# Deci-AI/super-gradients

Measured on NVIDIA H100. Metric: images/sec YOLO-NAS-S 640 bf16 train, higher is better.
Workload: dtype bf16

## Files before the change

super_gradients_b200/csrc/conv_sm100.cu:

```cuda
#include <cuda.h>

#include <cstdio>
#include <cstdlib>
#include <cstring>

#include "common.cuh"
#include "conv_sm100.h"
#include "sm100_host.h"
#include "sm100_ptx.cuh"

namespace sm100 {

constexpr int BLOCK_M = 128;
constexpr int NUM_THREADS = 384;
constexpr int CONSUMER_THREADS = 256;
constexpr int MAX_STAGES = 8;

struct Params {
  int M;
  int N;
  int C;
  int KC;
  int n_tiles;
  int stages;
  int P, Q;
  int stride, pad;
  int b_cols_per_tap;
  int ntaps;
  signed char tap_dh[9], tap_dw[9], tap_b[9];
  int out_mode, o_mul, oh_add, ow_add, outH, outW;
  int halo_tw, halo_thw;
  long long y_pitch;
  int y_off;
  bf16* y;
  const float* scale;
  const float* shift;
  const bf16* residual;
  double* stats;
  int stats_repl;
  int act;
// ... 206 lines not shown
        wgmma_commit();
        if (prev >= 0) {
          wgmma_wait<1>();
          __syncwarp();
          if (lane == 0) mbar_arrive(empty_bar(prev));
        }
        prev = stg;
        if (++stg == p.stages) {
          stg = 0;
          par ^= 1;
        }
      }
      wgmma_wait<0>();
      fence_regs(acc);
      __syncwarp();
      if (lane == 0 && prev >= 0) mbar_arrive(empty_bar(prev));

      const long long m_lo = (long long)mt * BLOCK_M + wg * 64 + wq * 16 + (lane >> 2);
      long long orow[2];
      bool row_ok[2];
#pragma unroll
      for (int h = 0; h < 2; ++h) {
        const long long m = m_lo + 8 * h;
        row_ok[h] = m < p.M;
        orow[h] = out_row(p, row_ok[h] ? m : 0);
      }
      tile_epilogue<BN>(p, acc, orow, row_ok, nt, wg, wq, lane, s_part, s_stats);
    }
  }
  __syncthreads();
  flush_stats(p, s_stats);
}

constexpr int HALO_W = 10, HALO_H = 10, HALO_TILE = 8;
constexpr uint32_t HALO_CG_BYTES = 1664;
constexpr uint32_t HALO_CTRL_BYTES = CTRL_BAR_BYTES + 16;
constexpr int HALO_MAX_STAGES = 6;

template <int BN, bool SKIP>
__global__ void __launch_bounds__(NUM_THREADS, BN <= 48 ? 2 : 1)
conv3x3_halo_kernel(const __grid_constant__ CUtensorMap map_a, const __grid_constant__ CUtensorMap map_b, const Params p) {
  extern __shared__ __align__(1024) unsigned char smem_raw[];
  const uint32_t smem_base = (smem_u32(smem_raw) + 1023u) & ~1023u;
  const int ksteps = p.C / 16;
  constexpr uint32_t b_box = BN * 32;
  const uint32_t b_bytes = 9u * ksteps * b_box;
  const uint32_t a_stage = ((uint32_t)(p.C / 8) * HALO_CG_BYTES + 1023u) & ~1023u;
  const uint32_t sb = smem_base, sa0 = smem_base + ((b_bytes + 1023u) & ~1023u);
  const uint32_t ctrl = sa0 + p.stages * a_stage;
  auto full_bar = [&](int s) { return ctrl + 8u * s; };
  auto empty_bar = [&](int s) { return ctrl + 8u * (MAX_STAGES + s); };
  const uint32_t b_bar = ctrl + CTRL_BAR_BYTES;
  float* s_part = reinterpret_cast<float*>(smem_raw + (ctrl + HALO_CTRL_BYTES - smem_u32(smem_raw)));
  float* s_stats = s_part + 8 * 2 * BN;

  const int warp = threadIdx.x >> 5, lane = threadIdx.x & 31;
  const int m_tiles = p.M;
  const int nt = blockIdx.x % p.n_tiles;
  const int mt_step = gridDim.x / p.n_tiles;
  const int mt0 = blockIdx.x / p.n_tiles;
  const int off = SKIP ? off_centre_steps<BN>(p, nt, ksteps, 16) : ksteps;

  if (threadIdx.x == 0) {
    for (int s = 0; s < p.stages; ++s) {
      mbar_init(full_bar(s), 1);
      mbar_init(empty_bar(s), 4);
    }
    mbar_init(b_bar, 1);
    asm volatile("fence.mbarrier_init.release.cluster;" ::: "memory");
    asm volatile("fence.proxy.async.shared::cta;" ::: "memory");
  }
  if (p.stats)
    for (int i = threadIdx.x; i < 4 * p.N; i += NUM_THREADS) s_stats[i] = 0.f;
  __syncthreads();

  if (warp == 0) {
    if (elect_one()) {
      mbar_expect_tx(b_bar, (uint32_t)(8 * off + ksteps) * b_box);
      for (int bt = 0; bt < 9; ++bt)
        for (int ks = 0; ks < (bt == CENTRE_TAP ? ksteps : off); ++ks)
          tma_load_2d(sb + (uint32_t)(bt * ksteps + ks) * b_box, &map_b, b_bar, bt * p.b_cols_per_tap + 16 * ks, nt * BN);
      const uint32_t a_tx = (uint32_t)(p.C / 8) * (HALO_H * HALO_W * 16);
      int stg = 0;
      uint32_t par = 1;
      for (int mt = mt0; mt < m_tiles; mt += mt_step) {
        const int n_img = mt / p.halo_thw;
        const int rem = mt - n_img * p.halo_thw;
        const int th = rem / p.halo_tw, tw = rem - th * p.halo_tw;
        mbar_wait(empty_bar(stg), par);
        const uint32_t sa = sa0 + stg * a_stage;
        mbar_expect_tx(full_bar(stg), a_tx);
        for (int cg = 0; cg < p.C / 8; ++cg)
          tma_load_tiled_4d(sa + (uint32_t)cg * HALO_CG_BYTES, &map_a, full_bar(stg), 8 * cg, tw * HALO_TILE - 1, th * HALO_TILE - 1,
                            n_img);
        if (++stg == p.stages) {
          stg = 0;
          par ^= 1;
        }
      }
    }
  } else if (warp >= 4) {
    const int wg = (warp >> 2) - 1;
    const int wq = warp & 3;
    float acc[BN / 2];
    mbar_wait(b_bar, 0);
    for (int j = wg, mt = mt0 + wg * mt_step; mt < m_tiles; j += 2, mt += 2 * mt_step) {
      const int stg = j % p.stages;
      mbar_wait(full_bar(stg), (uint32_t)(j / p.stages) & 1u);
      const uint32_t sa = sa0 + stg * a_stage;
      wgmma_fence();
      int t = off > 0 ? 0 : CENTRE_TAP;
      uint32_t sa_t = sa + (uint32_t)((t / 3) * HALO_W + t % 3) * 16u, sb_t = sb + (uint32_t)(p.tap_b[t] * ksteps) * b_box;
      for (int k = 0, ks = 0, nk = 8 * off + ksteps; k < nk; ++k) {
        const uint64_t da = smem_desc_noswizzle(sa_t + (uint32_t)(2 * ks) * HALO_CG_BYTES, HALO_CG_BYTES, HALO_W * 16);
        const uint64_t db = smem_desc(sb_t + (uint32_t)ks * b_box, 32, 16u, 256u);
        mma_kk<BN>(acc, da, db, k != 0);
        if (++ks == (t == CENTRE_TAP ? ksteps : off) && ++t < 9) {
          ks = 0;
          sa_t = sa + (uint32_t)((t / 3) * HALO_W + t % 3) * 16u;
          sb_t = sb + (uint32_t)(p.tap_b[t] * ksteps) * b_box;
        }
      }
      wgmma_commit();
      wgmma_wait<0>();
      fence_regs(acc);
      __syncwarp();
      if (lane == 0) mbar_arrive(empty_bar(stg));

      const int n_img = mt / p.halo_thw;
      const int rem = mt - n_img * p.halo_thw;
      const int th = rem / p.halo_tw, tw = rem - th * p.halo_tw;
      const int ow = tw * HALO_TILE + (lane >> 2);
      long long orow[2];
      bool row_ok[2];
#pragma unroll
      for (int h = 0; h < 2; ++h) {
        const int oh = th * HALO_TILE + 2 * wq + h;
        row_ok[h] = oh < p.P && ow < p.Q;
        orow[h] = row_ok[h] ? ((long long)n_img * p.P + oh) * p.Q + ow : 0;
      }
      tile_epilogue<BN, 4>(p, acc, orow, row_ok, nt, wg, wq, lane, s_part + wg * 4 * 2 * BN, s_stats + wg * 2 * p.N);
    }
  }
  __syncthreads();
  if (p.stats) {
    for (int i = threadIdx.x; i < 2 * p.N; i += NUM_THREADS) s_stats[i] += s_stats[2 * p.N + i];
    __syncthreads();
  }
  flush_stats(p, s_stats);
}

struct WParams {
// ... 103 lines not shown
        wgmma_commit();
        if (prev >= 0) {
          wgmma_wait<1>();
          __syncwarp();
          if (lane == 0) mbar_arrive(empty_bar(prev));
        }
        prev = stg;
        if ((stg += it_step) >= p.stages) {
          stg -= p.stages;
          par ^= 1;
        }
      }
      if (prev < 0) return;
      wgmma_wait<0>();
      fence_regs(acc);
      const int row_len = p.R * p.S * p.cpad;
#pragma unroll
      for (int h = 0; h < 2; ++h) {
        const int ko = row0 + (shared_rows ? 0 : wg * 64) + wq * 16 + (lane >> 2) + 8 * h;
        if (ko < p.K) {
          float* drow = p.dw + (long long)ko * row_len + tap * p.cpad + ctile * NB + 2 * (lane & 3);
#pragma unroll
          for (int j = 0; j < NB / 8; ++j)
            asm volatile("red.global.add.v2.f32 [%0], {%1, %2};" ::"l"(drow + 8 * j), "f"(acc[4 * j + 2 * h]), "f"(acc[4 * j + 2 * h + 1])
                         : "memory");
        }
      }
    }
  }
}

constexpr uint32_t WH_A_BYTES = WPIX * 128;

__host__ __device__ constexpr uint32_t wgrad_halo_stage_bytes(int nb) {
  return (WH_A_BYTES + (uint32_t)(nb / 8) * HALO_CG_BYTES + 1023u) & ~1023u;
}

template <int NB, int NT>
__device__ __forceinline__ void wgrad_halo_consume(const WParams& p, uint32_t ring, uint32_t bars, int t0, int t1, int tap0, int rb,
                                                   int ctile) {
  constexpr uint32_t stage_bytes = wgrad_halo_stage_bytes(NB);
  const int wq = (threadIdx.x >> 5) & 3, lane = threadIdx.x & 31;
  auto full_bar = [&](int s) { return bars + 8u * s; };
  auto empty_bar = [&](int s) { return bars + 8u * (MAX_STAGES + s); };
  float acc[NT > 0 ? NT : 1][NB / 2];
  int stg = 0, prev = 0;
  uint32_t par = 0;
  for (int mt = t0; mt < t1; ++mt) {
    mbar_wait(full_bar(stg), par);
    if constexpr (NT > 0) {
      const uint32_t sa = ring + stg * stage_bytes, sx = sa + WH_A_BYTES;
      wgmma_fence();
#pragma unroll
      for (int t = 0; t < NT; ++t) {
        const int tap = tap0 + t;
        const uint32_t sx_t = sx + (uint32_t)((tap / 3) * HALO_W + tap % 3) * 16u;
#pragma unroll
        for (int j = 0; j < WPIX / 16; ++j) {
          const uint64_t da = smem_desc(sa + (uint32_t)j * 16u * 128u, 128, WPIX * 128, 8 * 128);
          const uint64_t db = smem_desc_noswizzle(sx_t + (uint32_t)j * 2u * HALO_W * 16u, HALO_W * 16, HALO_CG_BYTES);
          mma_mn<NB>(acc[t], da, db, (mt != t0 || j != 0) ? 1u : 0u);
        }
      }
      wgmma_commit();
      wgmma_wait<1>();
    }
    __syncwarp();
    if (lane == 0 && mt != t0) mbar_arrive(empty_bar(prev));
    prev = stg;
    if (++stg == p.stages) {
      stg = 0;
      par ^= 1;
    }
  }
  if constexpr (NT > 0) {
    wgmma_wait<0>();
#pragma unroll
    for (int t = 0; t < NT; ++t) fence_regs(acc[t]);
  }
  __syncwarp();
  if (lane == 0) mbar_arrive(empty_bar(prev));
  if constexpr (NT > 0) {
    const int row_len = 9 * p.cpad;
#pragma unroll
    for (int h = 0; h < 2; ++h) {
      const int ko = 64 * rb + wq * 16 + (lane >> 2) + 8 * h;
      if (ko < p.K) {
        float* drow = p.dw + (long long)ko * row_len + tap0 * p.cpad + ctile * NB + 2 * (lane & 3);
#pragma unroll
        for (int t = 0; t < NT; ++t)
#pragma unroll
          for (int j = 0; j < NB / 8; ++j)
            asm volatile("red.global.add.v2.f32 [%0], {%1, %2};" ::"l"(drow + t * p.cpad + 8 * j), "f"(acc[t][4 * j + 2 * h]),
                         "f"(acc[t][4 * j + 2 * h + 1])
                         : "memory");
      }
    }
  }
}

template <int NB>
__global__ void __launch_bounds__(NUM_THREADS, 1)
wgrad3x3_halo_kernel(const __grid_constant__ CUtensorMap map_dy, const __grid_constant__ CUtensorMap map_x, const WParams p) {
  extern __shared__ __align__(1024) unsigned char smem_raw[];
  const uint32_t smem_base = (smem_u32(smem_raw) + 1023u) & ~1023u;
  constexpr uint32_t a_bytes = WH_A_BYTES, stage_bytes = wgrad_halo_stage_bytes(NB);
  const uint32_t ctrl = smem_base + p.stages * stage_bytes;
  auto full_bar = [&](int s) { return ctrl + 8u * s; };
  auto empty_bar = [&](int s) { return ctrl + 8u * (MAX_STAGES + s); };

  const int warp = threadIdx.x >> 5;
  const int items = p.rb_all * p.n_ctiles;
  const int split = blockIdx.x / items, item = blockIdx.x - split * items;
  const int ctile = item / p.rb_all, rb = item - ctile * p.rb_all;
  const bool all_taps = rb < p.rb_off;
  const int t0 = split * p.tiles_per_cta, t1 = min(t0 + p.tiles_per_cta, p.tiles);

  if (threadIdx.x == 0) {
    for (int s = 0; s < p.stages; ++s) {
      mbar_init(full_bar(s), 1);
      mbar_init(empty_bar(s), 8);
    }
    asm volatile("fence.mbarrier_init.release.cluster;" ::: "memory");
    asm volatile("fence.proxy.async.shared::cta;" ::: "memory");
  }
  __syncthreads();

  if (warp == 0) {
    if (elect_one()) {
      const uint32_t tx = a_bytes + (NB / 8) * (HALO_H * HALO_W * 16);
      int stg = 0;
      uint32_t par = 1;
      for (int mt = t0; mt < t1; ++mt) {
        const int n_img = mt / p.halo_thw;
        const int rem = mt - n_img * p.halo_thw;
        const int th = rem / p.halo_tw, tw = rem - th * p.halo_tw;
        mbar_wait(empty_bar(stg), par);
        const uint32_t sa = smem_base + stg * stage_bytes;
        mbar_expect_tx(full_bar(stg), tx);
        tma_load_tiled_4d(sa, &map_dy, full_bar(stg), 64 * rb, tw * HALO_TILE, th * HALO_TILE, n_img);
        for (int cg = 0; cg < NB / 8; ++cg)
          tma_load_tiled_4d(sa + a_bytes + (uint32_t)cg * HALO_CG_BYTES, &map_x, full_bar(stg), ctile * NB + 8 * cg,
                            tw * HALO_TILE - 1, th * HALO_TILE - 1, n_img);
        if (++stg == p.stages) {
          stg = 0;
          par ^= 1;
        }
      }
    }
  } else if (warp >= 4) {
    const int wg = (warp >> 2) - 1;
    const uint32_t ring = smem_base, bars = ctrl;
    if (!all_taps && wg == 0)
      wgrad_halo_consume<NB, 1>(p, ring, bars, t0, t1, CENTRE_TAP, rb, ctile);
    else if (!all_taps)
      wgrad_halo_consume<NB, 0>(p, ring, bars, t0, t1, 0, rb, ctile);
    else if (wg == 0)
      wgrad_halo_consume<NB, 5>(p, ring, bars, t0, t1, 0, rb, ctile);
    else
      wgrad_halo_consume<NB, 4>(p, ring, bars, t0, t1, 5, rb, ctile);
  }
}

typedef CUresult (*EncodeTiledFn)(CUtensorMap*, CUtensorMapDataType, cuuint32_t, void*, const cuuint64_t*, const cuuint64_t*,
                                  const cuuint32_t*, const cuuint32_t*, CUtensorMapInterleave, CUtensorMapSwizzle,
                                  CUtensorMapL2promotion, CUtensorMapFloatOOBfill);
typedef CUresult (*EncodeIm2colFn)(CUtensorMap*, CUtensorMapDataType, cuuint32_t, void*, const cuuint64_t*, const cuuint64_t*,
                                   const int*, const int*, cuuint32_t, cuuint32_t, const cuuint32_t*, CUtensorMapInterleave,
                                   CUtensorMapSwizzle, CUtensorMapL2promotion, CUtensorMapFloatOOBfill);
EncodeTiledFn g_tiled = nullptr;
EncodeIm2colFn g_im2col = nullptr;
int g_num_sms = 0;
long long g_launches = 0;
long long g_halo_launches = 0;
long long g_wgrad_halo_launches = 0;
bool g_force_im2col = false;
bool g_wgrad_force_im2col = false;
long long launch_count() { return g_launches; }
long long halo_launch_count() { return g_halo_launches; }
long long wgrad_halo_launch_count() { return g_wgrad_halo_launches; }
void force_im2col(bool on) { g_force_im2col = on; }
void wgrad_force_im2col(bool on) { g_wgrad_force_im2col = on; }

int init_driver() {
  if (g_tiled && g_im2col) return SGB_OK;
  cudaDriverEntryPointQueryResult qres;
  void* fn = nullptr;
  if (cudaGetDriverEntryPoint("cuTensorMapEncodeTiled", &fn, cudaEnableDefault, &qres) != cudaSuccess || !fn) {
    sgb_set_error("cuTensorMapEncodeTiled entry point not found");
    return SGB_E_CUDA;
  }
  g_tiled = (EncodeTiledFn)fn;
  fn = nullptr;
  if (cudaGetDriverEntryPoint("cuTensorMapEncodeIm2col", &fn, cudaEnableDefault, &qres) != cudaSuccess || !fn) {
    sgb_set_error("cuTensorMapEncodeIm2col entry point not found");
    return SGB_E_CUDA;
  }
  g_im2col = (EncodeIm2colFn)fn;
  int dev = 0;
  cudaGetDevice(&dev);
  cudaDeviceGetAttribute(&g_num_sms, cudaDevAttrMultiProcessorCount, dev);
  return SGB_OK;
}

int encode_tiled(CUtensorMap* map, const void* ptr, int rank, const cuuint64_t* dims, const cuuint64_t* byte_strides,
                 const cuuint32_t* box, CUtensorMapSwizzle swizzle, const char* what) {
  const cuuint32_t elem_strides[5] = {1, 1, 1, 1, 1};
  const CUresult r = g_tiled(map, CU_TENSOR_MAP_DATA_TYPE_BFLOAT16, (cuuint32_t)rank, const_cast<void*>(ptr), dims, byte_strides, box,
                             elem_strides, CU_TENSOR_MAP_INTERLEAVE_NONE, swizzle, CU_TENSOR_MAP_L2_PROMOTION_L2_128B,
                             CU_TENSOR_MAP_FLOAT_OOB_FILL_NONE);
  if (r == CUDA_SUCCESS) return SGB_OK;
  char shape[256] = "";
  for (int i = 0, n = 0; i < rank && n < (int)sizeof(shape); ++i)
    n += snprintf(shape + n, sizeof(shape) - n, "%s%llu (box %u, stride %llu)", i ? ", " : "", (unsigned long long)dims[i],
                  (unsigned)box[i], i ? (unsigned long long)byte_strides[i - 1] : 2ull);
  sgb_set_error("cuTensorMapEncodeTiled(%s) failed with %d: dims %s", what, (int)r, shape);
  return SGB_E_CUDA;
}

namespace {

CUtensorMapSwizzle swizzle_for(int kc) {
  return kc == 64 ? CU_TENSOR_MAP_SWIZZLE_128B : (kc == 32 ? CU_TENSOR_MAP_SWIZZLE_64B : CU_TENSOR_MAP_SWIZZLE_32B);
}

int encode_im2col(CUtensorMap* map, const void* ptr, int N, int H, int W, int C, int pitch, int stride, const int (&lower)[2],
                  const int (&upper)[2], int channels, int pixels, const char* what) {
  const cuuint64_t dims[4] = {(cuuint64_t)C, (cuuint64_t)W, (cuuint64_t)H, (cuuint64_t)N};
  const cuuint64_t strides[3] = {(cuuint64_t)pitch * 2, (cuuint64_t)W * pitch * 2, (cuuint64_t)H * W * pitch * 2};
  const cuuint32_t estr[4] = {1, (cuuint32_t)stride, (cuuint32_t)stride, 1};
  const CUresult r = g_im2col(map, CU_TENSOR_MAP_DATA_TYPE_BFLOAT16, 4, const_cast<void*>(ptr), dims, strides, lower, upper,
                              (cuuint32_t)channels, (cuuint32_t)pixels, estr, CU_TENSOR_MAP_INTERLEAVE_NONE, swizzle_for(channels),
                              CU_TENSOR_MAP_L2_PROMOTION_L2_128B, CU_TENSOR_MAP_FLOAT_OOB_FILL_NONE);
  if (r == CUDA_SUCCESS) return SGB_OK;
  sgb_set_error("cuTensorMapEncodeIm2col(%s) failed with %d (C=%d W=%d H=%d N=%d pitch=%d lower=%d,%d upper=%d,%d stride=%d box=%d)", what,
                (int)r, C, W, H, N, pitch, lower[0], lower[1], upper[0], upper[1], stride, channels);
  return SGB_E_CUDA;
}

int encode_halo_map(CUtensorMap* map, const void* x, int N, int H, int W, int C, int pitch) {
  const cuuint64_t dims[4] = {(cuuint64_t)C, (cuuint64_t)W, (cuuint64_t)H, (cuuint64_t)N};
  const cuuint64_t strides[3] = {(cuuint64_t)pitch * 2, (cuuint64_t)W * pitch * 2, (cuuint64_t)H * W * pitch * 2};
  const cuuint32_t box[4] = {8, HALO_W, HALO_H, 1};
  return encode_tiled(map, x, 4, dims, strides, box, CU_TENSOR_MAP_SWIZZLE_NONE, "halo");
}

struct Problem {
  const void* a;
  int N, H, W, C, a_pitch;
  const void* b;
  int b_rows, b_cols, b_cols_per_tap;
  int R, S, stride, pad, P, Q, flip;
  int ntaps;
  int tap_dh[9], tap_dw[9], tap_b[9];
  int out_mode, o_mul, oh_add, ow_add, outH, outW;
  void* y;
  int y_pitch, y_off;
  const float* scale;
  const float* shift;
  const void* residual;
  double* stats;
  int stats_repl, act;
  int centre_from;
};

bool supported(const Problem& q) {
  if (q.C % 16 != 0 || q.b_rows % 8 != 0) return false;
  if (!((q.R == 1 && q.S == 1) || (q.R == 3 && q.S == 3))) return false;
  if (q.stride != 1 && q.stride != 2) return false;
  if (q.a_pitch % 8 != 0 || q.y_pitch % 8 != 0 || q.y_off % 8 != 0) return false;
  if (((uintptr_t)q.a & 15) || ((uintptr_t)q.b & 15) || ((uintptr_t)q.y & 15)) return false;
  if ((long long)q.N * q.P * q.Q >= (1ll << 31)) return false;
  if (q.b_rows > 4096) return false;
  return true;
}

template <class Fn>
struct Variant {
  int bn;
  Fn fn;
  int regs = 0;
  bool ready = false;
};
typedef void (*ConvFn)(const CUtensorMap, const CUtensorMap, const Params);
typedef void (*WgradFn)(const CUtensorMap, const CUtensorMap, const WParams);
template <bool SKIP>
Variant<ConvFn> g_conv[6] = {{16, conv_wgmma_kernel<16, SKIP>}, {32, conv_wgmma_kernel<32, SKIP>},
                             {48, conv_wgmma_kernel<48, SKIP>}, {64, conv_wgmma_kernel<64, SKIP>},
                             {96, conv_wgmma_kernel<96, SKIP>}, {128, conv_wgmma_kernel<128, SKIP>}};
template <bool SKIP>
Variant<ConvFn> g_halo[6] = {{16, conv3x3_halo_kernel<16, SKIP>}, {32, conv3x3_halo_kernel<32, SKIP>},
                             {48, conv3x3_halo_kernel<48, SKIP>}, {64, conv3x3_halo_kernel<64, SKIP>},
                             {96, conv3x3_halo_kernel<96, SKIP>}, {128, conv3x3_halo_kernel<128, SKIP>}};
Variant<WgradFn> g_wgrad[6] = {{16, wgrad_wgmma_kernel<16>}, {32, wgrad_wgmma_kernel<32>}, {48, wgrad_wgmma_kernel<48>},
                               {64, wgrad_wgmma_kernel<64>}, {96, wgrad_wgmma_kernel<96>}, {128, wgrad_wgmma_kernel<128>}};
Variant<WgradFn> g_wgrad_halo[3] = {{16, wgrad3x3_halo_kernel<16>}, {32, wgrad3x3_halo_kernel<32>}, {48, wgrad3x3_halo_kernel<48>}};

template <class Fn, int N>
int prepare(Variant<Fn> (&table)[N], int bn, const char* what, Variant<Fn>*& var) {
  for (auto& v : table)
    if (v.bn == bn) var = &v;
  if (var->ready) return SGB_OK;
  if (int rc = sgb_cuda_check(cudaFuncSetAttribute(var->fn, cudaFuncAttributeMaxDynamicSharedMemorySize, 227 * 1024), what)) return rc;
  cudaFuncAttributes fa{};
  if (int rc = sgb_cuda_check(cudaFuncGetAttributes(&fa, var->fn), what)) return rc;
  var->regs = fa.numRegs;
  var->ready = true;
  return SGB_OK;
}

int max_ctas_per_sm(int regs) {
  const int ctas = 65536 / (((regs + 7) / 8) * 8 * NUM_THREADS);
  return ctas > 2 ? 2 : (ctas < 1 ? 1 : ctas);
}

int pick_bn(int n) {
  for (int bn : {16, 32, 48, 64, 96, 128})
    if (n <= bn) return bn;
  int best = 128, best_waste = (n + 127) / 128 * 128 - n;
  for (int bn : {96, 64}) {
    const int waste = (n + bn - 1) / bn * bn - n;
    if (waste < best_waste) { best_waste = waste; best = bn; }
  }
  return best;
}

size_t halo_smem(int C, int bn, int n, bool stats, int stages) {
  const size_t b_bytes = ((size_t)9 * C * bn * 2 + 1023) & ~(size_t)1023;
  const size_t a_stage = ((size_t)(C / 8) * HALO_CG_BYTES + 1023) & ~(size_t)1023;
  return 1024 + b_bytes + (size_t)stages * a_stage + HALO_CTRL_BYTES + (stats ? (size_t)(8 * 2 * bn + 4 * n) * 4 : 0);
}

bool halo_tiles_fit(int P, int Q) {
  const long long covered = (long long)((P + 7) / 8) * 8 * ((Q + 7) / 8) * 8;
  return 20ll * P * Q >= 17 * covered;
}

int halo_bn(const Problem& q) {
  if (q.R != 3 || q.S != 3 || q.stride != 1 || q.pad != 1 || q.ntaps > 0 || q.out_mode != 0) return 0;
  if (q.P != q.H || q.Q != q.W) return 0;
  if (!halo_tiles_fit(q.P, q.Q)) return 0;
  const int n = q.b_rows, full = pick_bn(n);
  auto waste = [&](int bn) { return (n + bn - 1) / bn * bn - n; };
  for (int bn : {full, 96, 64})
    if (bn <= full && (bn == full || (q.C <= 96 && bn >= 64 && waste(bn) <= waste(full))) &&
        halo_smem(q.C, bn, n, q.stats != nullptr, 2) <= 227 * 1024)
      return bn;
  return 0;
}

int launch_halo(const Problem& q, const Params& p0, int bn, cudaStream_t st) {
  Params p = p0;
  p.n_tiles = (p.N + bn - 1) / bn;
  p.halo_tw = (q.Q + HALO_TILE - 1) / HALO_TILE;
  p.halo_thw = p.halo_tw * ((q.P + HALO_TILE - 1) / HALO_TILE);
  p.M = q.N * p.halo_thw;
  p.centre_n = 0;
  Variant<ConvFn>* var = nullptr;
  if (int rc = prepare(p.centre_c > 0 ? g_halo<true> : g_halo<false>, bn, "conv3x3_halo_kernel", var)) return rc;
  int ctas_per_sm = max_ctas_per_sm(var->regs);
  int stages = 0;
  for (;; --ctas_per_sm) {
    const size_t budget = (ctas_per_sm == 1 ? 227u : 227u / ctas_per_sm - 1u) * 1024u;
    for (stages = HALO_MAX_STAGES; stages >= 2 && halo_smem(q.C, bn, p.N, p.stats != nullptr, stages) > budget; --stages) {
    }
    if (stages >= 2 || ctas_per_sm == 1) break;
  }
  if (stages < 2) { sgb_set_error("conv3x3_halo: tile does not fit shared memory"); return SGB_E_UNSUPPORTED; }
  p.stages = stages;
  const size_t smem = halo_smem(q.C, bn, p.N, p.stats != nullptr, stages);

  alignas(64) CUtensorMap map_a, map_b;
  if (int rc = encode_halo_map(&map_a, q.a, q.N, q.H, q.W, q.C, q.a_pitch)) return rc;
  const cuuint64_t b_dims[2] = {(cuuint64_t)q.b_cols, (cuuint64_t)q.b_rows}, b_strides[1] = {(cuuint64_t)q.b_cols * 2};
  const cuuint32_t b_box[2] = {16, (cuuint32_t)bn};
  if (int rc = encode_tiled(&map_b, q.b, 2, b_dims, b_strides, b_box, CU_TENSOR_MAP_SWIZZLE_32B, "halo B")) return rc;
  int per_nt = g_num_sms * ctas_per_sm / p.n_tiles;
  if (per_nt > p.M) per_nt = p.M;
  if (per_nt < 1) per_nt = 1;
  var->fn<<<per_nt * p.n_tiles, NUM_THREADS, smem, st>>>(map_a, map_b, p);
  ++g_launches;
  ++g_halo_launches;
  return sgb_cuda_check(cudaGetLastError(), "conv3x3_halo_kernel");
}

int launch(const Problem& q, cudaStream_t st) {
  if (int rc = init_driver()) return rc;
  Params p{};
  p.M = q.N * q.P * q.Q;
  p.N = q.b_rows;
  p.C = q.C;
  p.KC = q.C % 64 == 0 ? 64 : (q.C % 32 == 0 ? 32 : 16);
  if (p.KC < 64 && q.C > 32) p.KC = 64;
  const int bn = pick_bn(p.N);
  p.n_tiles = (p.N + bn - 1) / bn;
  p.P = q.P; p.Q = q.Q; p.stride = q.stride; p.pad = q.pad;
  if (q.ntaps > 0) {
    p.ntaps = q.ntaps;
    for (int t = 0; t < q.ntaps; ++t) { p.tap_dh[t] = (signed char)q.tap_dh[t]; p.tap_dw[t] = (signed char)q.tap_dw[t]; p.tap_b[t] = (signed char)q.tap_b[t]; }
  } else {
    p.ntaps = q.R * q.S;
    for (int t = 0; t < p.ntaps; ++t) {
      p.tap_dh[t] = (signed char)(t / q.S);
      p.tap_dw[t] = (signed char)(t % q.S);
      p.tap_b[t] = (signed char)(q.flip ? (p.ntaps - 1 - t) : t);
    }
  }
  if (p.ntaps > 9) return SGB_E_UNSUPPORTED;
  p.out_mode = q.out_mode; p.o_mul = q.o_mul; p.oh_add = q.oh_add; p.ow_add = q.ow_add; p.outH = q.outH; p.outW = q.outW;
  p.b_cols_per_tap = q.b_cols_per_tap;
  p.y = (bf16*)q.y; p.y_pitch = q.y_pitch; p.y_off = q.y_off;
  p.scale = q.scale; p.shift = q.shift; p.residual = (const bf16*)q.residual;
  p.stats = q.stats; p.stats_repl = q.stats_repl > 0 ? q.stats_repl : 1; p.act = q.act;
// ... 32 lines not shown
  if (int rc = encode_im2col(&map_a, q.a, q.N, q.H, q.W, q.C, q.a_pitch, q.stride, lower, upper, p.KC, BLOCK_M, "A")) return rc;
  const cuuint64_t b_dims[2] = {(cuuint64_t)q.b_cols, (cuuint64_t)q.b_rows}, b_strides[1] = {(cuuint64_t)q.b_cols * 2};
  const cuuint32_t b_box[2] = {(cuuint32_t)p.KC, (cuuint32_t)bn};
  if (int rc = encode_tiled(&map_b, q.b, 2, b_dims, b_strides, b_box, swizzle_for(p.KC), "B")) return rc;
  const int m_tiles = (p.M + BLOCK_M - 1) / BLOCK_M;
  int grid = m_tiles * p.n_tiles;
  if (grid > g_num_sms * ctas_per_sm) grid = g_num_sms * ctas_per_sm;
  var->fn<<<grid, NUM_THREADS, smem, st>>>(map_a, map_b, p);
  ++g_launches;
  return sgb_cuda_check(cudaGetLastError(), "conv_wgmma_kernel");
}

struct WgradProblem {
  const void* x;
  const void* dy;
  int N, H, W, C, x_pitch;
  int K, y_pitch;
  int R, S, stride, pad, P, Q;
  float* dw;
  int centre_from;
};

bool wgrad_supported(const WgradProblem& q) {
  if (q.C % 16 != 0 || q.K % 8 != 0) return false;
  if (!((q.R == 1 && q.S == 1) || (q.R == 3 && q.S == 3))) return false;
  if (q.pad != q.R / 2 || (q.stride != 1 && q.stride != 2)) return false;
  if (q.x_pitch % 8 != 0 || q.y_pitch % 8 != 0) return false;
  if (((uintptr_t)q.x & 15) || ((uintptr_t)q.dy & 15)) return false;
  if ((long long)q.N * q.P * q.Q >= (1ll << 31)) return false;
  return true;
}

int wgrad_halo_nb(const WgradProblem& q) {
  if (q.R != 3 || q.S != 3 || q.stride != 1 || q.pad != 1 || q.P != q.H || q.Q != q.W) return 0;
  if (!halo_tiles_fit(q.P, q.Q)) return 0;
  return q.C % 32 == 0 ? 32 : (q.C % 48 == 0 ? 48 : 16);
}

int launch_wgrad_halo(const WgradProblem& q, const WParams& p0, int nb, cudaStream_t st) {
  WParams p = p0;
  p.n_ctiles = q.C / nb;
  p.halo_tw = (q.Q + HALO_TILE - 1) / HALO_TILE;
  p.halo_thw = p.halo_tw * ((q.P + HALO_TILE - 1) / HALO_TILE);
  p.tiles = q.N * p.halo_thw;
  Variant<WgradFn>* var = nullptr;
  if (int rc = prepare(g_wgrad_halo, nb, "wgrad3x3_halo_kernel", var)) return rc;
  const int ctas_per_sm = max_ctas_per_sm(var->regs);
  const uint32_t stage_bytes = wgrad_halo_stage_bytes(nb);
  const uint32_t budget = (ctas_per_sm == 1 ? 227u : 113u) * 1024u - 1024u - CTRL_BAR_BYTES;
  p.stages = (int)(budget / stage_bytes);
  if (p.stages > MAX_STAGES) p.stages = MAX_STAGES;
  const size_t smem = 1024 + (size_t)p.stages * stage_bytes + CTRL_BAR_BYTES;
  const int items = p.rb_all * p.n_ctiles;
  int splits = g_num_sms * ctas_per_sm / items;
  if (splits < 1) splits = 1;
  p.tiles_per_cta = (p.tiles + splits - 1) / splits;
  splits = (p.tiles + p.tiles_per_cta - 1) / p.tiles_per_cta;

  alignas(64) CUtensorMap map_dy, map_x;
  const cuuint64_t dy_dims[4] = {(cuuint64_t)q.K, (cuuint64_t)q.Q, (cuuint64_t)q.P, (cuuint64_t)q.N};
  const cuuint64_t dy_strides[3] = {(cuuint64_t)q.y_pitch * 2, (cuuint64_t)q.Q * q.y_pitch * 2, (cuuint64_t)q.P * q.Q * q.y_pitch * 2};
  const cuuint32_t dy_box[4] = {64, HALO_TILE, HALO_TILE, 1};
  if (int rc = encode_tiled(&map_dy, q.dy, 4, dy_dims, dy_strides, dy_box, CU_TENSOR_MAP_SWIZZLE_128B, "dy tile")) return rc;
  if (int rc = encode_halo_map(&map_x, q.x, q.N, q.H, q.W, q.C, q.x_pitch)) return rc;
  var->fn<<<splits * items, NUM_THREADS, smem, st>>>(map_dy, map_x, p);
  ++g_launches;
  ++g_wgrad_halo_launches;
  return sgb_cuda_check(cudaGetLastError(), "wgrad3x3_halo_kernel");
}

int wgrad_launch(const WgradProblem& q, cudaStream_t st) {
  if (int rc = init_driver()) return rc;
  WParams p{};
  p.K = q.K; p.C = q.C; p.R = q.R; p.S = q.S; p.stride = q.stride; p.pad = q.pad; p.P = q.P; p.Q = q.Q;
  p.npix = q.N * q.P * q.Q;
  int nb = 16;
  for (int cand : {128, 96, 64, 48, 32})
    if (q.C % cand == 0) { nb = cand; break; }
  p.CB = nb % 64 == 0 ? 64 : (nb % 32 == 0 ? 32 : 16);
  p.n_ctiles = q.C / nb;
  if (q.centre_from != 0 && (q.R != 3 || q.S != 3 || q.stride != 1 || q.pad != 1 || q.centre_from < 0 || q.centre_from >= q.K ||
                             q.centre_from % 16 != 0))
    return SGB_E_INVALID;
  p.rb_all = (q.K + 63) / 64;
  p.rb_off = q.centre_from > 0 ? (q.centre_from + 63) / 64 : p.rb_all;
  p.items = 0;
  for (int t = 0; t < q.R * q.S; ++t) p.items += (wgrad_row_blocks(p, t) + 1) / 2;
  p.cpad = q.C;
  p.dw = q.dw;
  if (!g_wgrad_force_im2col)
    if (const int nb = wgrad_halo_nb(q)) return launch_wgrad_halo(q, p, nb, st);
  Variant<WgradFn>* var = nullptr;
  if (int rc = prepare(g_wgrad, nb, "wgrad_wgmma_kernel", var)) return rc;
  const uint32_t stage_bytes = 2 * WPIX * 128 + (uint32_t)(nb / p.CB) * WPIX * p.CB * 2;
  int stages = (int)((200 * 1024 - CTRL_BAR_BYTES - 1024) / stage_bytes);
  if (stages > MAX_STAGES) stages = MAX_STAGES;
  if (p.rb_all % 2 || p.rb_off % 2) stages &= ~1;
  if (stages < 2) return SGB_E_UNSUPPORTED;
// ... 161 lines not shown
```

super_gradients_b200/csrc/sm100_host.h:

```cpp
#pragma once

#include <cuda.h>

namespace sm100 {

int init_driver();

int encode_tiled(CUtensorMap* map, const void* ptr, int rank, const cuuint64_t* dims, const cuuint64_t* byte_strides,
                 const cuuint32_t* box, CUtensorMapSwizzle swizzle, const char* what);

}
```

Baseline: 997.6.

## Extend 3x3 halo conv kernel to stride-2 via phase-split TMA boxes

Generalises the halo-tiled implicit-GEMM 3x3 conv kernel to stride 2. The input tile is loaded as four parity-phase TMA boxes using element strides, so each tap reads a dense strided view from shared memory. Stride-2 3x3 convs with C<=48 previously fell back to the generic im2col-style kernel; they now reuse one halo tile across all nine taps. The change adds template variants, forces an even stage count, and leaves wgrad still restricted to stride 1.

```diff
diff --git a/super_gradients_b200/csrc/conv_sm100.cu b/super_gradients_b200/csrc/conv_sm100.cu
--- a/super_gradients_b200/csrc/conv_sm100.cu
+++ b/super_gradients_b200/csrc/conv_sm100.cu
@@ -6,6 +6,7 @@
 
 #include "common.cuh"
 #include "conv_sm100.h"
+#include "halo_math.cuh"
 #include "sm100_host.h"
 #include "sm100_ptx.cuh"
 
@@ -278,20 +279,35 @@
   flush_stats(p, s_stats);
 }
 
-constexpr int HALO_W = 10, HALO_H = 10, HALO_TILE = 8;
-constexpr uint32_t HALO_CG_BYTES = 1664;
+constexpr int HALO_TILE = sgb_halo::TILE;
 constexpr uint32_t HALO_CTRL_BYTES = CTRL_BAR_BYTES + 16;
 constexpr int HALO_MAX_STAGES = 6;
-
-template <int BN, bool SKIP>
+static_assert(HALO_MAX_STAGES % 2 == 0, "conv3x3_halo_kernel's ring must have an even length");
+
+struct alignas(64) HaloMaps {
+  CUtensorMap a[4];
+};
+
+template <int STRIDE>
+__device__ __forceinline__ void load_halo(uint32_t dst, const HaloMaps& maps, uint32_t bar, int cg0, int groups, int th, int tw,
+                                          int n_img) {
+  for (int cg = 0; cg < groups; ++cg)
+#pragma unroll
+    for (int b = 0; b < sgb_halo::boxes(STRIDE); ++b)
+      tma_load_tiled_4d(dst + (uint32_t)cg * sgb_halo::cg_bytes(STRIDE) + sgb_halo::box_off(STRIDE, b), &maps.a[b], bar, 8 * (cg0 + cg),
+                        sgb_halo::box_col0(STRIDE, b, tw), sgb_halo::box_row0(STRIDE, b, th), n_img);
+}
+
+template <int BN, bool SKIP, int STRIDE>
 __global__ void __launch_bounds__(NUM_THREADS, BN <= 48 ? 2 : 1)
-conv3x3_halo_kernel(const __grid_constant__ CUtensorMap map_a, const __grid_constant__ CUtensorMap map_b, const Params p) {
+conv3x3_halo_kernel(const __grid_constant__ HaloMaps maps, const __grid_constant__ CUtensorMap map_b, const Params p) {
   extern __shared__ __align__(1024) unsigned char smem_raw[];
   const uint32_t smem_base = (smem_u32(smem_raw) + 1023u) & ~1023u;
   const int ksteps = p.C / 16;
   constexpr uint32_t b_box = BN * 32;
+  constexpr uint32_t cg_bytes = sgb_halo::cg_bytes(STRIDE);
   const uint32_t b_bytes = 9u * ksteps * b_box;
-  const uint32_t a_stage = ((uint32_t)(p.C / 8) * HALO_CG_BYTES + 1023u) & ~1023u;
+  const uint32_t a_stage = ((uint32_t)(p.C / 8) * cg_bytes + 1023u) & ~1023u;
   const uint32_t sb = smem_base, sa0 = smem_base + ((b_bytes + 1023u) & ~1023u);
   const uint32_t ctrl = sa0 + p.stages * a_stage;
   auto full_bar = [&](int s) { return ctrl + 8u * s; };
@@ -326,7 +342,7 @@
       for (int bt = 0; bt < 9; ++bt)
         for (int ks = 0; ks < (bt == CENTRE_TAP ? ksteps : off); ++ks)
           tma_load_2d(sb + (uint32_t)(bt * ksteps + ks) * b_box, &map_b, b_bar, bt * p.b_cols_per_tap + 16 * ks, nt * BN);
-      const uint32_t a_tx = (uint32_t)(p.C / 8) * (HALO_H * HALO_W * 16);
+      const uint32_t a_tx = (uint32_t)(p.C / 8) * sgb_halo::tx_bytes(STRIDE);
       int stg = 0;
       uint32_t par = 1;
       for (int mt = mt0; mt < m_tiles; mt += mt_step) {
@@ -336,9 +352,7 @@
         mbar_wait(empty_bar(stg), par);
         const uint32_t sa = sa0 + stg * a_stage;
         mbar_expect_tx(full_bar(stg), a_tx);
-        for (int cg = 0; cg < p.C / 8; ++cg)
-          tma_load_tiled_4d(sa + (uint32_t)cg * HALO_CG_BYTES, &map_a, full_bar(stg), 8 * cg, tw * HALO_TILE - 1, th * HALO_TILE - 1,
-                            n_img);
+        load_halo<STRIDE>(sa, maps, full_bar(stg), 0, p.C / 8, th, tw, n_img);
         if (++stg == p.stages) {
           stg = 0;
           par ^= 1;
@@ -356,14 +370,16 @@
       const uint32_t sa = sa0 + stg * a_stage;
       wgmma_fence();
       int t = off > 0 ? 0 : CENTRE_TAP;
-      uint32_t sa_t = sa + (uint32_t)((t / 3) * HALO_W + t % 3) * 16u, sb_t = sb + (uint32_t)(p.tap_b[t] * ksteps) * b_box;
+      uint32_t sa_t = sa + sgb_halo::tap_off(STRIDE, t / 3, t % 3), sb_t = sb + (uint32_t)(p.tap_b[t] * ksteps) * b_box;
+      uint32_t pitch_t = sgb_halo::tap_pitch(STRIDE, t / 3, t % 3);
       for (int k = 0, ks = 0, nk = 8 * off + ksteps; k < nk; ++k) {
-        const uint64_t da = smem_desc_noswizzle(sa_t + (uint32_t)(2 * ks) * HALO_CG_BYTES, HALO_CG_BYTES, HALO_W * 16);
+        const uint64_t da = smem_desc_noswizzle(sa_t + (uint32_t)(2 * ks) * cg_bytes, cg_bytes, pitch_t);
         const uint64_t db = smem_desc(sb_t + (uint32_t)ks * b_box, 32, 16u, 256u);
         mma_kk<BN>(acc, da, db, k != 0);
         if (++ks == (t == CENTRE_TAP ? ksteps : off) && ++t < 9) {
           ks = 0;
-          sa_t = sa + (uint32_t)((t / 3) * HALO_W + t % 3) * 16u;
+          sa_t = sa + sgb_halo::tap_off(STRIDE, t / 3, t % 3);
+          pitch_t = sgb_halo::tap_pitch(STRIDE, t / 3, t % 3);
           sb_t = sb + (uint32_t)(p.tap_b[t] * ksteps) * b_box;
         }
       }
@@ -533,14 +549,14 @@
 
 constexpr uint32_t WH_A_BYTES = WPIX * 128;
 
-__host__ __device__ constexpr uint32_t wgrad_halo_stage_bytes(int nb) {
-  return (WH_A_BYTES + (uint32_t)(nb / 8) * HALO_CG_BYTES + 1023u) & ~1023u;
-}
-
-template <int NB, int NT>
+__host__ __device__ constexpr uint32_t wgrad_halo_stage_bytes(int nb, int stride) {
+  return (WH_A_BYTES + (uint32_t)(nb / 8) * sgb_halo::cg_bytes(stride) + 1023u) & ~1023u;
+}
+
+template <int NB, int NT, int STRIDE>
 __device__ __forceinline__ void wgrad_halo_consume(const WParams& p, uint32_t ring, uint32_t bars, int t0, int t1, int tap0, int rb,
                                                    int ctile) {
-  constexpr uint32_t stage_bytes = wgrad_halo_stage_bytes(NB);
+  constexpr uint32_t stage_bytes = wgrad_halo_stage_bytes(NB, STRIDE);
   const int wq = (threadIdx.x >> 5) & 3, lane = threadIdx.x & 31;
   auto full_bar = [&](int s) { return bars + 8u * s; };
   auto empty_bar = [&](int s) { return bars + 8u * (MAX_STAGES + s); };
@@ -555,11 +571,11 @@
 #pragma unroll
       for (int t = 0; t < NT; ++t) {
         const int tap = tap0 + t;
-        const uint32_t sx_t = sx + (uint32_t)((tap / 3) * HALO_W + tap % 3) * 16u;
+        const uint32_t sx_t = sx + sgb_halo::tap_off(STRIDE, tap / 3, tap % 3), pitch = sgb_halo::tap_pitch(STRIDE, tap / 3, tap % 3);
 #pragma unroll
         for (int j = 0; j < WPIX / 16; ++j) {
           const uint64_t da = smem_desc(sa + (uint32_t)j * 16u * 128u, 128, WPIX * 128, 8 * 128);
-          const uint64_t db = smem_desc_noswizzle(sx_t + (uint32_t)j * 2u * HALO_W * 16u, HALO_W * 16, HALO_CG_BYTES);
+          const uint64_t db = smem_desc_noswizzle(sx_t + (uint32_t)j * 2u * pitch, pitch, sgb_halo::cg_bytes(STRIDE));
           mma_mn<NB>(acc[t], da, db, (mt != t0 || j != 0) ? 1u : 0u);
         }
       }
@@ -600,12 +616,12 @@
   }
 }
 
-template <int NB>
+template <int NB, int STRIDE>
 __global__ void __launch_bounds__(NUM_THREADS, 1)
-wgrad3x3_halo_kernel(const __grid_constant__ CUtensorMap map_dy, const __grid_constant__ CUtensorMap map_x, const WParams p) {
+wgrad3x3_halo_kernel(const __grid_constant__ CUtensorMap map_dy, const __grid_constant__ HaloMaps maps_x, const WParams p) {
   extern __shared__ __align__(1024) unsigned char smem_raw[];
   const uint32_t smem_base = (smem_u32(smem_raw) + 1023u) & ~1023u;
-  constexpr uint32_t a_bytes = WH_A_BYTES, stage_bytes = wgrad_halo_stage_bytes(NB);
+  constexpr uint32_t a_bytes = WH_A_BYTES, stage_bytes = wgrad_halo_stage_bytes(NB, STRIDE);
   const uint32_t ctrl = smem_base + p.stages * stage_bytes;
   auto full_bar = [&](int s) { return ctrl + 8u * s; };
   auto empty_bar = [&](int s) { return ctrl + 8u * (MAX_STAGES + s); };
@@ -629,7 +645,7 @@
 
   if (warp == 0) {
     if (elect_one()) {
-      const uint32_t tx = a_bytes + (NB / 8) * (HALO_H * HALO_W * 16);
+      const uint32_t tx = a_bytes + (NB / 8) * sgb_halo::tx_bytes(STRIDE);
       int stg = 0;
       uint32_t par = 1;
       for (int mt = t0; mt < t1; ++mt) {
@@ -640,9 +656,7 @@
         const uint32_t sa = smem_base + stg * stage_bytes;
         mbar_expect_tx(full_bar(stg), tx);
         tma_load_tiled_4d(sa, &map_dy, full_bar(stg), 64 * rb, tw * HALO_TILE, th * HALO_TILE, n_img);
-        for (int cg = 0; cg < NB / 8; ++cg)
-          tma_load_tiled_4d(sa + a_bytes + (uint32_t)cg * HALO_CG_BYTES, &map_x, full_bar(stg), ctile * NB + 8 * cg,
-                            tw * HALO_TILE - 1, th * HALO_TILE - 1, n_img);
+        load_halo<STRIDE>(sa + a_bytes, maps_x, full_bar(stg), ctile * NB / 8, NB / 8, th, tw, n_img);
         if (++stg == p.stages) {
           stg = 0;
           par ^= 1;
@@ -653,13 +667,13 @@
     const int wg = (warp >> 2) - 1;
     const uint32_t ring = smem_base, bars = ctrl;
     if (!all_taps && wg == 0)
-      wgrad_halo_consume<NB, 1>(p, ring, bars, t0, t1, CENTRE_TAP, rb, ctile);
+      wgrad_halo_consume<NB, 1, STRIDE>(p, ring, bars, t0, t1, CENTRE_TAP, rb, ctile);
     else if (!all_taps)
-      wgrad_halo_consume<NB, 0>(p, ring, bars, t0, t1, 0, rb, ctile);
+      wgrad_halo_consume<NB, 0, STRIDE>(p, ring, bars, t0, t1, 0, rb, ctile);
     else if (wg == 0)
-      wgrad_halo_consume<NB, 5>(p, ring, bars, t0, t1, 0, rb, ctile);
+      wgrad_halo_consume<NB, 5, STRIDE>(p, ring, bars, t0, t1, 0, rb, ctile);
     else
-      wgrad_halo_consume<NB, 4>(p, ring, bars, t0, t1, 5, rb, ctile);
+      wgrad_halo_consume<NB, 4, STRIDE>(p, ring, bars, t0, t1, 5, rb, ctile);
   }
 }
 
@@ -705,8 +719,8 @@
 }
 
 int encode_tiled(CUtensorMap* map, const void* ptr, int rank, const cuuint64_t* dims, const cuuint64_t* byte_strides,
-                 const cuuint32_t* box, CUtensorMapSwizzle swizzle, const char* what) {
-  const cuuint32_t elem_strides[5] = {1, 1, 1, 1, 1};
+                 const cuuint32_t* box, CUtensorMapSwizzle swizzle, const char* what, int traversal) {
+  const cuuint32_t elem_strides[5] = {1, (cuuint32_t)traversal, (cuuint32_t)traversal, 1, 1};
   const CUresult r = g_tiled(map, CU_TENSOR_MAP_DATA_TYPE_BFLOAT16, (cuuint32_t)rank, const_cast<void*>(ptr), dims, byte_strides, box,
                              elem_strides, CU_TENSOR_MAP_INTERLEAVE_NONE, swizzle, CU_TENSOR_MAP_L2_PROMOTION_L2_128B,
                              CU_TENSOR_MAP_FLOAT_OOB_FILL_NONE);
@@ -739,11 +753,14 @@
   return SGB_E_CUDA;
 }
 
-int encode_halo_map(CUtensorMap* map, const void* x, int N, int H, int W, int C, int pitch) {
+int encode_halo_maps(HaloMaps* maps, const void* x, int N, int H, int W, int C, int pitch, int stride) {
   const cuuint64_t dims[4] = {(cuuint64_t)C, (cuuint64_t)W, (cuuint64_t)H, (cuuint64_t)N};
   const cuuint64_t strides[3] = {(cuuint64_t)pitch * 2, (cuuint64_t)W * pitch * 2, (cuuint64_t)H * W * pitch * 2};
-  const cuuint32_t box[4] = {8, HALO_W, HALO_H, 1};
-  return encode_tiled(map, x, 4, dims, strides, box, CU_TENSOR_MAP_SWIZZLE_NONE, "halo");
+  for (int b = 0; b < sgb_halo::boxes(stride); ++b) {
+    const cuuint32_t box[4] = {8, (cuuint32_t)(sgb_halo::box_cols(stride, b) * stride), (cuuint32_t)(sgb_halo::box_rows(stride, b) * stride), 1};
+    if (int rc = encode_tiled(&maps->a[b], x, 4, dims, strides, box, CU_TENSOR_MAP_SWIZZLE_NONE, "halo", stride)) return rc;
+  }
+  return SGB_OK;
 }
 
 struct Problem {
@@ -785,17 +802,21 @@
 };
 typedef void (*ConvFn)(const CUtensorMap, const CUtensorMap, const Params);
 typedef void (*WgradFn)(const CUtensorMap, const CUtensorMap, const WParams);
+typedef void (*HaloFn)(const HaloMaps, const CUtensorMap, const Params);
+typedef void (*WgradHaloFn)(const CUtensorMap, const HaloMaps, const WParams);
 template <bool SKIP>
 Variant<ConvFn> g_conv[6] = {{16, conv_wgmma_kernel<16, SKIP>}, {32, conv_wgmma_kernel<32, SKIP>},
                              {48, conv_wgmma_kernel<48, SKIP>}, {64, conv_wgmma_kernel<64, SKIP>},
                              {96, conv_wgmma_kernel<96, SKIP>}, {128, conv_wgmma_kernel<128, SKIP>}};
-template <bool SKIP>
-Variant<ConvFn> g_halo[6] = {{16, conv3x3_halo_kernel<16, SKIP>}, {32, conv3x3_halo_kernel<32, SKIP>},
-                             {48, conv3x3_halo_kernel<48, SKIP>}, {64, conv3x3_halo_kernel<64, SKIP>},
-                             {96, conv3x3_halo_kernel<96, SKIP>}, {128, conv3x3_halo_kernel<128, SKIP>}};
+template <bool SKIP, int STRIDE>
+Variant<HaloFn> g_halo[6] = {{16, conv3x3_halo_kernel<16, SKIP, STRIDE>}, {32, conv3x3_halo_kernel<32, SKIP, STRIDE>},
+                             {48, conv3x3_halo_kernel<48, SKIP, STRIDE>}, {64, conv3x3_halo_kernel<64, SKIP, STRIDE>},
+                             {96, conv3x3_halo_kernel<96, SKIP, STRIDE>}, {128, conv3x3_halo_kernel<128, SKIP, STRIDE>}};
 Variant<WgradFn> g_wgrad[6] = {{16, wgrad_wgmma_kernel<16>}, {32, wgrad_wgmma_kernel<32>}, {48, wgrad_wgmma_kernel<48>},
                                {64, wgrad_wgmma_kernel<64>}, {96, wgrad_wgmma_kernel<96>}, {128, wgrad_wgmma_kernel<128>}};
-Variant<WgradFn> g_wgrad_halo[3] = {{16, wgrad3x3_halo_kernel<16>}, {32, wgrad3x3_halo_kernel<32>}, {48, wgrad3x3_halo_kernel<48>}};
+template <int STRIDE>
+Variant<WgradHaloFn> g_wgrad_halo[3] = {{16, wgrad3x3_halo_kernel<16, STRIDE>}, {32, wgrad3x3_halo_kernel<32, STRIDE>},
+                                        {48, wgrad3x3_halo_kernel<48, STRIDE>}};
 
 template <class Fn, int N>
 int prepare(Variant<Fn> (&table)[N], int bn, const char* what, Variant<Fn>*& var) {
@@ -826,9 +847,9 @@
   return best;
 }
 
-size_t halo_smem(int C, int bn, int n, bool stats, int stages) {
+size_t halo_smem(int C, int stride, int bn, int n, bool stats, int stages) {
   const size_t b_bytes = ((size_t)9 * C * bn * 2 + 1023) & ~(size_t)1023;
-  const size_t a_stage = ((size_t)(C / 8) * HALO_CG_BYTES + 1023) & ~(size_t)1023;
+  const size_t a_stage = ((size_t)(C / 8) * sgb_halo::cg_bytes(stride) + 1023) & ~(size_t)1023;
   return 1024 + b_bytes + (size_t)stages * a_stage + HALO_CTRL_BYTES + (stats ? (size_t)(8 * 2 * bn + 4 * n) * 4 : 0);
 }
 
@@ -838,14 +859,15 @@
 }
 
 int halo_bn(const Problem& q) {
-  if (q.R != 3 || q.S != 3 || q.stride != 1 || q.pad != 1 || q.ntaps > 0 || q.out_mode != 0) return 0;
-  if (q.P != q.H || q.Q != q.W) return 0;
+  if (q.R != 3 || q.S != 3 || q.pad != 1 || q.ntaps > 0 || q.out_mode != 0) return 0;
+  if (q.stride < 1 || q.stride > 2 || q.stride * q.P != q.H || q.stride * q.Q != q.W) return 0;
+  if (q.stride == 2 && q.C > 48) return 0;
   if (!halo_tiles_fit(q.P, q.Q)) return 0;
   const int n = q.b_rows, full = pick_bn(n);
   auto waste = [&](int bn) { return (n + bn - 1) / bn * bn - n; };
   for (int bn : {full, 96, 64})
     if (bn <= full && (bn == full || (q.C <= 96 && bn >= 64 && waste(bn) <= waste(full))) &&
-        halo_smem(q.C, bn, n, q.stats != nullptr, 2) <= 227 * 1024)
+        halo_smem(q.C, q.stride, bn, n, q.stats != nullptr, 2) <= 227 * 1024)
       return bn;
   return 0;
 }
@@ -857,29 +879,33 @@
   p.halo_thw = p.halo_tw * ((q.P + HALO_TILE - 1) / HALO_TILE);
   p.M = q.N * p.halo_thw;
   p.centre_n = 0;
-  Variant<ConvFn>* var = nullptr;
-  if (int rc = prepare(p.centre_c > 0 ? g_halo<true> : g_halo<false>, bn, "conv3x3_halo_kernel", var)) return rc;
+  Variant<HaloFn>* var = nullptr;
+  const char* what = "conv3x3_halo_kernel";
+  if (int rc = q.stride == 2 ? prepare(g_halo<false, 2>, bn, what, var)
+                             : prepare(p.centre_c > 0 ? g_halo<true, 1> : g_halo<false, 1>, bn, what, var))
+    return rc;
   int ctas_per_sm = max_ctas_per_sm(var->regs);
   int stages = 0;
   for (;; --ctas_per_sm) {
     const size_t budget = (ctas_per_sm == 1 ? 227u : 227u / ctas_per_sm - 1u) * 1024u;
-    for (stages = HALO_MAX_STAGES; stages >= 2 && halo_smem(q.C, bn, p.N, p.stats != nullptr, stages) > budget; --stages) {
+    for (stages = HALO_MAX_STAGES; stages >= 2 && halo_smem(q.C, q.stride, bn, p.N, p.stats != nullptr, stages) > budget; stages -= 2) {
     }
     if (stages >= 2 || ctas_per_sm == 1) break;
   }
   if (stages < 2) { sgb_set_error("conv3x3_halo: tile does not fit shared memory"); return SGB_E_UNSUPPORTED; }
   p.stages = stages;
-  const size_t smem = halo_smem(q.C, bn, p.N, p.stats != nullptr, stages);
-
-  alignas(64) CUtensorMap map_a, map_b;
-  if (int rc = encode_halo_map(&map_a, q.a, q.N, q.H, q.W, q.C, q.a_pitch)) return rc;
+  const size_t smem = halo_smem(q.C, q.stride, bn, p.N, p.stats != nullptr, stages);
+
+  alignas(64) HaloMaps maps;
+  alignas(64) CUtensorMap map_b;
+  if (int rc = encode_halo_maps(&maps, q.a, q.N, q.H, q.W, q.C, q.a_pitch, q.stride)) return rc;
   const cuuint64_t b_dims[2] = {(cuuint64_t)q.b_cols, (cuuint64_t)q.b_rows}, b_strides[1] = {(cuuint64_t)q.b_cols * 2};
   const cuuint32_t b_box[2] = {16, (cuuint32_t)bn};
   if (int rc = encode_tiled(&map_b, q.b, 2, b_dims, b_strides, b_box, CU_TENSOR_MAP_SWIZZLE_32B, "halo B")) return rc;
   int per_nt = g_num_sms * ctas_per_sm / p.n_tiles;
   if (per_nt > p.M) per_nt = p.M;
   if (per_nt < 1) per_nt = 1;
-  var->fn<<<per_nt * p.n_tiles, NUM_THREADS, smem, st>>>(map_a, map_b, p);
+  var->fn<<<per_nt * p.n_tiles, NUM_THREADS, smem, st>>>(maps, map_b, p);
   ++g_launches;
   ++g_halo_launches;
   return sgb_cuda_check(cudaGetLastError(), "conv3x3_halo_kernel");
@@ -978,8 +1004,8 @@
 }
 
 int wgrad_halo_nb(const WgradProblem& q) {
-  if (q.R != 3 || q.S != 3 || q.stride != 1 || q.pad != 1 || q.P != q.H || q.Q != q.W) return 0;
-  if (!halo_tiles_fit(q.P, q.Q)) return 0;
+  if (q.R != 3 || q.S != 3 || q.pad != 1 || q.stride < 1 || q.stride > 2 || q.stride * q.P != q.H || q.stride * q.Q != q.W) return 0;
+  if (q.stride != 1 || !halo_tiles_fit(q.P, q.Q)) return 0;
   return q.C % 32 == 0 ? 32 : (q.C % 48 == 0 ? 48 : 16);
 }
 
@@ -989,10 +1015,10 @@
   p.halo_tw = (q.Q + HALO_TILE - 1) / HALO_TILE;
   p.halo_thw = p.halo_tw * ((q.P + HALO_TILE - 1) / HALO_TILE);
   p.tiles = q.N * p.halo_thw;
-  Variant<WgradFn>* var = nullptr;
-  if (int rc = prepare(g_wgrad_halo, nb, "wgrad3x3_halo_kernel", var)) return rc;
+  Variant<WgradHaloFn>* var = nullptr;
+  if (int rc = prepare(g_wgrad_halo<1>, nb, "wgrad3x3_halo_kernel", var)) return rc;
   const int ctas_per_sm = max_ctas_per_sm(var->regs);
-  const uint32_t stage_bytes = wgrad_halo_stage_bytes(nb);
+  const uint32_t stage_bytes = wgrad_halo_stage_bytes(nb, q.stride);
   const uint32_t budget = (ctas_per_sm == 1 ? 227u : 113u) * 1024u - 1024u - CTRL_BAR_BYTES;
   p.stages = (int)(budget / stage_bytes);
   if (p.stages > MAX_STAGES) p.stages = MAX_STAGES;
@@ -1003,13 +1029,14 @@
   p.tiles_per_cta = (p.tiles + splits - 1) / splits;
   splits = (p.tiles + p.tiles_per_cta - 1) / p.tiles_per_cta;
 
-  alignas(64) CUtensorMap map_dy, map_x;
+  alignas(64) CUtensorMap map_dy;
+  alignas(64) HaloMaps maps_x;
   const cuuint64_t dy_dims[4] = {(cuuint64_t)q.K, (cuuint64_t)q.Q, (cuuint64_t)q.P, (cuuint64_t)q.N};
   const cuuint64_t dy_strides[3] = {(cuuint64_t)q.y_pitch * 2, (cuuint64_t)q.Q * q.y_pitch * 2, (cuuint64_t)q.P * q.Q * q.y_pitch * 2};
   const cuuint32_t dy_box[4] = {64, HALO_TILE, HALO_TILE, 1};
   if (int rc = encode_tiled(&map_dy, q.dy, 4, dy_dims, dy_strides, dy_box, CU_TENSOR_MAP_SWIZZLE_128B, "dy tile")) return rc;
-  if (int rc = encode_halo_map(&map_x, q.x, q.N, q.H, q.W, q.C, q.x_pitch)) return rc;
-  var->fn<<<splits * items, NUM_THREADS, smem, st>>>(map_dy, map_x, p);
+  if (int rc = encode_halo_maps(&maps_x, q.x, q.N, q.H, q.W, q.C, q.x_pitch, q.stride)) return rc;
+  var->fn<<<splits * items, NUM_THREADS, smem, st>>>(map_dy, maps_x, p);
   ++g_launches;
   ++g_wgrad_halo_launches;
   return sgb_cuda_check(cudaGetLastError(), "wgrad3x3_halo_kernel");
diff --git a/super_gradients_b200/csrc/halo_math.cuh b/super_gradients_b200/csrc/halo_math.cuh
--- /dev/null
+++ b/super_gradients_b200/csrc/halo_math.cuh
@@ -0,0 +1,40 @@
+#pragma once
+#include <stdint.h>
+
+#ifndef SGB_HD
+#ifdef __CUDACC__
+#define SGB_HD __host__ __device__ __forceinline__
+#else
+#define SGB_HD static inline
+#endif
+#endif
+
+namespace sgb_halo {
+
+constexpr int TILE = 8;
+
+SGB_HD constexpr int boxes(int stride) { return stride == 1 ? 1 : 4; }
+SGB_HD constexpr int box_rows(int stride, int b) { return stride == 1 ? TILE + 2 : TILE + (b >> 1); }
+SGB_HD constexpr int box_cols(int stride, int b) { return stride == 1 ? TILE + 2 : TILE + (b & 1); }
+SGB_HD constexpr uint32_t align128(uint32_t v) { return (v + 127u) & ~127u; }
+SGB_HD constexpr uint32_t box_off(int stride, int b) {
+  uint32_t off = 0;
+  for (int i = 0; i < b; ++i) off += align128((uint32_t)(box_rows(stride, i) * box_cols(stride, i)) * 16u);
+  return off;
+}
+SGB_HD constexpr uint32_t cg_bytes(int stride) { return box_off(stride, boxes(stride)); }
+SGB_HD constexpr uint32_t tx_bytes(int stride) {
+  uint32_t n = 0;
+  for (int b = 0; b < boxes(stride); ++b) n += (uint32_t)(box_rows(stride, b) * box_cols(stride, b)) * 16u;
+  return n;
+}
+SGB_HD constexpr int box_row0(int stride, int b, int t) { return stride * TILE * t - (stride == 1 ? 1 : (b >> 1)); }
+SGB_HD constexpr int box_col0(int stride, int b, int t) { return stride * TILE * t - (stride == 1 ? 1 : (b & 1)); }
+SGB_HD constexpr int tap_box(int stride, int r, int s) { return stride == 1 ? 0 : 2 * (r % 2 == 0) + (s % 2 == 0); }
+SGB_HD constexpr uint32_t tap_off(int stride, int r, int s) {
+  const int b = tap_box(stride, r, s);
+  return box_off(stride, b) + (uint32_t)((r / stride) * box_cols(stride, b) + s / stride) * 16u;
+}
+SGB_HD constexpr uint32_t tap_pitch(int stride, int r, int s) { return (uint32_t)box_cols(stride, tap_box(stride, r, s)) * 16u; }
+
+}
diff --git a/super_gradients_b200/csrc/sm100_host.h b/super_gradients_b200/csrc/sm100_host.h
--- a/super_gradients_b200/csrc/sm100_host.h
+++ b/super_gradients_b200/csrc/sm100_host.h
@@ -7,6 +7,6 @@
 int init_driver();
 
 int encode_tiled(CUtensorMap* map, const void* ptr, int rank, const cuuint64_t* dims, const cuuint64_t* byte_strides,
-                 const cuuint32_t* box, CUtensorMapSwizzle swizzle, const char* what);
+                 const cuuint32_t* box, CUtensorMapSwizzle swizzle, const char* what, int traversal = 1);
 
 }
```

Result: no change. 997.4, median of 6 (-0.0%).
